# pappuks/medical-image-codec

Hardware: AMD Instinct MI355X
Metric: PICS-8 encode+decode throughput over raw u16 bytes (XR-shaped frames), lossless (higher is better)
Workload: dtype u16; 1 GPU; PICS-8 encode+decode, 288 distinct XR-like 2577x2048 12-bit synthetic frames (2304 strips) per GPU per step, noise tuned to the published XR PICS-8 ratio; frames_per_gpu=288, strips_per_frame=8, width=2577, height=2048, fse=2-state (CompressParallelStrips default), parallelism=1 x independent batches

## Files before the change

### medical-image-codec_amd/csrc/mic_api.hip

```cpp
#include "mic_session.h"

namespace micapi {

std::mutex g_mu;
std::condition_variable g_pool_cv;
int g_device = 0;
std::vector<int> g_devices(1, 0);
bool g_device_ok = false;
std::string g_device_name;
struct DevPool { std::vector<mic_hip_session *> free_; int made = 0; };
std::map<int, DevPool> g_pools;
thread_local mic_hip_session *tl_default = nullptr;
thread_local int tl_depth = 0;

static int pool_max() {
    static const int v = [] { const char *e = getenv("MIC_HIP_POOL"); const int n = e ? atoi(e) : 3; return std::min(std::max(n, 1), 16); }();
    return v;
}

int check_device(int device) {
    static std::mutex mu; static std::vector<int8_t> known;
    std::lock_guard<std::mutex> lk(mu);
    int n = 0;
    if (device < 0 || hipGetDeviceCount(&n) != hipSuccess || device >= n) return MIC_ERR_DEVICE;
// ... 585 lines not shown
    out8[0] = u.ntok; out8[1] = u.blob_len; out8[2] = u.table_log; out8[3] = u.symbol_len;
    out8[4] = u.max_count; out8[5] = u.hdr_len; out8[6] = u.zero_bits; out8[7] = u.flavour;
    out8[8] = u.count; out8[9] = u.bits_off; out8[10] = (uint32_t)u.nstates_used; out8[11] = (uint32_t)u.status; out8[12] = u.nseg; out8[13] = u.nsym; out8[14] = u.seg_cap;
    out8[15] = u.dec_kernel;
    for (int k = 0; k < 16; k++) out8[16 + k] = u.dbg[k];
    return MIC_OK;
} MIC_ABI_CATCH
int mic_hip_debug_split(mic_hip_session *s, int i, uint32_t *out) try {
    if (!s || !out || i < 0 || i >= s->n_last) return MIC_ERR_ARGS;
    for (int k = 0; k < 3; k++) out[k] = s->h_units[(size_t)i].split[k];
    return MIC_OK;
} MIC_ABI_CATCH
int mic_hip_debug_split_config(mic_hip_session *s, uint32_t min_tokens, uint32_t overlap, uint32_t min_bits16) try {
    if (!s || (overlap && (overlap < 64u || (overlap & 63u)))) return MIC_ERR_ARGS;
    if (min_tokens) s->split_cfg.min_tokens = min_tokens;
    if (overlap) s->split_cfg.overlap = overlap;
    if (min_bits16) s->split_cfg.min_bits16 = min_bits16;
    s->dec_classes = mic_hip_session::ClsMemory{};
    return MIC_OK;
} MIC_ABI_CATCH
int mic_hip_debug_split4(mic_hip_session *s, int i, uint32_t *out) try {
    if (!s || !out || i < 0 || i >= s->n_last) return MIC_ERR_ARGS;
    const uint32_t *r = s->h_units[(size_t)i].split;
    const uint32_t m = r[7] == 4u ? ~0u : 0u;
    out[0] = r[0]; out[1] = r[1] & m; out[2] = r[3] & m; out[3] = r[4] & m; out[4] = r[2]; out[5] = r[5] & m; out[6] = r[6] & m;
    return MIC_OK;
} MIC_ABI_CATCH
int mic_hip_debug_split4_config(mic_hip_session *s, uint32_t min_tokens4) try {
    if (!s) return MIC_ERR_ARGS;
    if (min_tokens4) s->split_cfg.min_tokens4 = min_tokens4;
    s->dec_classes = mic_hip_session::ClsMemory{};
    return MIC_OK;
} MIC_ABI_CATCH
int mic_hip_debug_dec_cls(uint32_t flavour, uint32_t table_log, uint32_t zero_bits) { return mic_dec_cls(flavour, table_log, zero_bits); }
int mic_hip_debug_fetch_hist(mic_hip_session *s, int i, void *dst, size_t bytes) try {
    if (!s || i < 0 || i >= s->n_last || bytes > kSym * 4) return MIC_ERR_ARGS;
    HIP_TRY(hipMemcpy(dst, s->h_units[(size_t)i].hist, bytes, hipMemcpyDeviceToHost));
    return MIC_OK;
} MIC_ABI_CATCH
int mic_hip_debug_tok_paths(mic_hip_session *s, int i, uint32_t *out) try {
    if (!s || !out || i < 0 || i >= s->n_last) return MIC_ERR_ARGS;
    for (int k = 0; k < MIC_TK_PATHS; k++) out[k] = s->h_units[(size_t)i].tk_paths[k];
    return MIC_OK;
} MIC_ABI_CATCH
int mic_hip_debug_fetch_tok(mic_hip_session *s, int i, void *dst, size_t n) try {
    if (!s || i < 0 || i >= s->n_last || n > s->h_units[(size_t)i].tok_cap) return MIC_ERR_ARGS;
    HIP_TRY(hipMemcpy(dst, s->h_units[(size_t)i].tok, n * 2, hipMemcpyDeviceToHost));
    return MIC_OK;
} MIC_ABI_CATCH
int mic_hip_debug_tab_route(mic_hip_session *s, int i, uint32_t *out) try {
    if (!s || !out || i < 0 || i >= s->n_last) return MIC_ERR_ARGS;
    *out = s->h_units[(size_t)i].tb_route;
    return MIC_OK;
} MIC_ABI_CATCH
int mic_hip_debug_enc_kernel(mic_hip_session *s, int i, uint32_t *out) try {
    if (!s || !out || i < 0 || i >= s->n_last) return MIC_ERR_ARGS;
    const MicUnit &u = s->h_units[(size_t)i];
    out[0] = u.enc_kernel & 0xFFu; out[1] = u.enc_rounds; out[2] = (u.enc_kernel & MIC_ENC_HANDED) ? 1u : 0u;
    return MIC_OK;
} MIC_ABI_CATCH
int mic_hip_debug_fetch_table(mic_hip_session *s, int i, int which, void *dst, size_t bytes) try {
    if (!s || !dst || i < 0 || i >= s->n_last || which < 0 || which > 4) return MIC_ERR_ARGS;
    const MicUnit &u = s->h_units[(size_t)i];
    const void *slabs[5] = { u.state_tab, u.tt_nb, u.tt_find, u.tab_sym, u.norm };
    if (bytes > (size_t)u.tab_cap * (which == 3 ? 2 : 4)) return MIC_ERR_ARGS;
    { const int arc = s->activate(); if (arc) return arc; }
// ... 81 lines not shown
```

### medical-image-codec_amd/csrc/mic_decode_ls.hip

```cpp
#include <type_traits>
#include "mic_dev.h"
#include "mic_launch.h"
#include "mic_wave.h"
#include "mic_rlewalk.h"

#define LS_RING 0u
#define LS_CLASSES MIC_CLS_CLASSES
template <int TL> struct LsGeom {
    static constexpr int SPW = TL <= 12 ? 4 : TL == 13 ? 3 : TL == 14 ? 2 : 1;
    static constexpr int WAVES = TL <= 12 ? 4 : TL == 13 ? 3 : TL == 16 ? 1 : 2;
    static constexpr int RING_BLOCKS = TL == 16 ? 8 : 4;
    static constexpr int DEPTH = TL == 16 ? 3 : 2;
    static constexpr int RING_BITS = TL == 16 ? 9 : 8;
    static constexpr uint32_t MIRROR = 256u * RING_BLOCKS;
    static constexpr uint32_t STAGE = MIRROR + 16u;
    static constexpr uint32_t TAB = STAGE + 256u;
    static constexpr uint32_t STREAM_BYTES = TAB + (2u << TL);
    static constexpr uint32_t LDS = WAVES * SPW * STREAM_BYTES;
    static_assert(LDS <= 160 * 1024, "one group must fit a CU's LDS");
};
#define LS_TL 13

typedef __attribute__((address_space(3))) uint32_t *ls_l32;
typedef __attribute__((address_space(3))) uint16_t *ls_l16;
typedef const __attribute__((address_space(1))) uint16_t *ls_gcu16;
typedef const __attribute__((address_space(1))) uint32_t *ls_gcu32;
typedef __attribute__((address_space(1))) uint16_t *ls_gu16;
typedef __attribute__((address_space(1))) uint32_t *ls_gu32;
typedef uint32_t ls_v2 __attribute__((ext_vector_type(2)));

template <int CTRL> __device__ __forceinline__ uint32_t ls_dpp(uint32_t v) {
    return (uint32_t)__builtin_amdgcn_update_dpp(0, (int)v, CTRL, 0xF, 0xF, true);
}
#define LS_QP(a, b, c, d) ((a) | ((b) << 2) | ((c) << 4) | ((d) << 6))
#define LS_ROW_SHR(n) (0x110 + (n))
#define LS_ROW_HALF_MIRROR 0x141

__device__ __forceinline__ uint32_t ls_rl(uint32_t v, int lane) { return (uint32_t)__builtin_amdgcn_readlane((int)v, lane); }
__device__ __forceinline__ uint64_t ls_rl64(uint64_t v, int lane) {
    return ((uint64_t)ls_rl((uint32_t)(v >> 32), lane) << 32) | ls_rl((uint32_t)v, lane);
}

#define LS_SPLIT_LIST MIC_CLS_CLASSES
#define LS_RETRY_LIST (MIC_CLS_CLASSES + 1)
#define LS_SPLIT4_LIST (MIC_CLS_CLASSES + 2)
#define LS_LISTS MIC_CLS_LISTS
__global__ void __launch_bounds__(1024) k_dec_classify(MicUnit *units, int n, int *list, int *count, int split, MicSplitCfg cfg) {
    __shared__ uint32_t s_w[16][LS_LISTS];
    __shared__ uint32_t s_base[LS_LISTS];
    const uint32_t tid = threadIdx.x, lane = tid & 63, wave = tid >> 6;
    if (tid < LS_LISTS) s_base[tid] = 0;
    __syncthreads();
    for (int i0 = 0; i0 < n; i0 += 1024) {
        const int i = i0 + (int)tid;
        int cls = -1;
        if (i < n) {
            MicUnit &u = units[i];
            const uint32_t flav = u.flavour, tl = u.table_log;
            const uint32_t ns = (flav == 108) ? 8u : flav;
            if (u.status == MICD_OK && u.ntok == 0 && (ns == 2 || ns == 4 || ns == 8) && tl >= MIC_MIN_TABLELOG && tl <= MIC_MAX_TABLELOG &&
                !(tl == 16 && u.zero_bits)) {
                if (u.bits_off >= u.comp_len) u.status = MICD_ERR_CORRUPT;
                else if (u.comp_len - u.bits_off < (1u << 27)) {
                    if (u.comp_in[u.comp_len - 1] == 0) u.status = MICD_ERR_CORRUPT;
                    else {
                        cls = mic_dec_cls(flav, tl, u.zero_bits);
                        if (cls == 0 && split && mic_split_gate(u, cfg)) cls = u.count >= cfg.min_tokens4 ? LS_SPLIT4_LIST : LS_SPLIT_LIST;
                    }
                }
            }
        }
        uint32_t rank = 0;
#pragma unroll
        for (int c = 0; c < LS_LISTS; c++) {
            const uint64_t m = __ballot(cls == c);
            if (cls == c) rank = (uint32_t)__popcll(m & ((1ull << lane) - 1ull));
            if (lane == 0) s_w[wave][c] = (uint32_t)__popcll(m);
        }
        __syncthreads();
        if (cls >= 0) {
            uint32_t off = s_base[cls];
            for (uint32_t w = 0; w < wave; w++) off += s_w[w][cls];
            list[(size_t)cls * (size_t)n + off + rank] = i;
        }
        __syncthreads();
        if (tid < LS_LISTS) { uint32_t t = 0; for (int w = 0; w < 16; w++) t += s_w[w][tid]; s_base[tid] += t; }
        __syncthreads();
    }
    if (tid < LS_LISTS) count[tid] = (int)s_base[tid];
    if (tid == LS_RETRY_LIST) count[tid] = 0;
}

template <int N, bool ZB, int TL>
__global__ void __launch_bounds__(64 * LsGeom<TL>::WAVES) k_dec_tans_ls(MicUnit *units, const int *list, const int *count_p) {
    constexpr int LS_SPW = LsGeom<TL>::SPW, LS_WAVES = LsGeom<TL>::WAVES;
    constexpr uint32_t LS_STREAM_BYTES = LsGeom<TL>::STREAM_BYTES, LS_STAGE = LsGeom<TL>::STAGE, LS_TAB = LsGeom<TL>::TAB, LS_MIRROR = LsGeom<TL>::MIRROR;
    constexpr int LS_RB = LsGeom<TL>::RING_BLOCKS, LS_DEPTH = LsGeom<TL>::DEPTH, LS_RBITS = LsGeom<TL>::RING_BITS;
    extern __shared__ uint32_t s_mem[];
    const uint32_t lane = threadIdx.x & 63, wv = threadIdx.x >> 6;
    if ((uint32_t)(uintptr_t)(__attribute__((address_space(3))) uint32_t *)s_mem != 0u) return;
// ... 305 lines not shown
            const uint32_t hi = window(q - (int32_t)pre);
            const uint32_t nx = (uint32_t)((((uint64_t)e << 32) | hi) >> (32u - nb));
            st = valid ? nx : st;
            q += (int32_t)ntot;
        }
        __builtin_amdgcn_s_waitcnt(0xC07F);
#pragma unroll
        for (int j = 0; j < LS_SPW; j++) {
            if (!s_have[j]) continue;
            const uint32_t rj = ls_rl(rem, j * LS_LS), done = s_chunks[j] * 128u;
            const uint32_t s2 = *(ls_l32)(uintptr_t)((wv * LS_SPW + (uint32_t)j) * LS_STREAM_BYTES + LS_STAGE + lane * 4);
            const ls_gu16 o = (ls_gu16)(uintptr_t)s_out[j];
            if (2 * lane < rj) o[done + 2 * lane] = (uint16_t)s2;
            if (2 * lane + 1 < rj) o[done + 2 * lane + 1] = (uint16_t)(s2 >> 16);
        }
    }
    if (have && lane % LS_LS == 0 && lane < LS_SPW * LS_LS) {
        MicUnit &uo = units[list[slot0 + (int)g]];
        uo.dec_kernel = 1u + (uint32_t)((TL <= 12 ? 4 : TL - 13) * 6 + (N == 2 ? 0 : N == 4 ? 2 : 4) + (ZB ? 1 : 0));
        if (count == uo.count && q + 32 - (int32_t)(8u * sb) < 0) uo.status = MICD_ERR_CORRUPT;
        else { uo.ntok = count; uo.dec_stage = MIC_STAGE_STATES; }
    }
}

#ifdef LS_STAMP
#define LS_ST_DECL uint64_t stamp[5] = { 0, 0, 0, 0, 0 }, t_prev = __builtin_amdgcn_s_memtime()
#define LS_ST_OUT(parts_) do { if (lane == 0) { MicUnit &ud = units[unit_i]; for (int i_ = 0; i_ < 5; i_++) ud.dbg[i_] = (uint32_t)(stamp[i_] >> 4); \
                                                ud.dbg[5] = ch_end; ud.dbg[6] = (parts_); } } while (0)
#else
#define LS_ST_DECL do { } while (0)
#define LS_ST_OUT(parts_) do { } while (0)
#endif
template <int PARTS> struct LsParts {
    static_assert(PARTS == 2 || PARTS == 4, "eight parts do not fit the sym slab (DESIGN.md section 4)");
    static constexpr int TL = 13, SPW = 3, WAVES = 3;
    static constexpr int CHUNK = 128 / PARTS;
    static constexpr int BLK = 64 / PARTS, BLK_SHIFT = PARTS == 2 ? 5 : 4;
    static constexpr int RING_BLOCKS = 4, DEPTH = 2, RING_BITS = BLK_SHIFT + 2;
    static constexpr uint32_t MIRROR = 4u * BLK * RING_BLOCKS;
    static constexpr uint32_t STAGE = MIRROR + 16u;
    static constexpr uint32_t PART_BYTES = STAGE + 2u * CHUNK;
    static constexpr uint32_t TAB = (uint32_t)PARTS * PART_BYTES;
    static constexpr uint32_t STREAM_BYTES = TAB + (2u << TL);
    static constexpr uint32_t LDS = WAVES * SPW * STREAM_BYTES;
    static_assert(LDS <= 160 * 1024, "one group must fit a CU's LDS");
    static __device__ __forceinline__ uint32_t region(uint32_t sym_cap, uint32_t tok_cap, uint32_t T) {
        const uint32_t slab = min(sym_cap, tok_cap);
        return (PARTS == 2 ? min(slab, T) : slab / (uint32_t)(PARTS - 1)) & ~(uint32_t)(CHUNK - 1);
    }
};

template <int PARTS>
__global__ void __launch_bounds__(64 * LsParts<PARTS>::WAVES) k_dec_tans_ls_parts(MicUnit *units, const int *list, const int *count_p, int *retry_list,
                                                                                int *retry_count, uint32_t overlap) {
    using G = LsParts<PARTS>;
    constexpr int LS_SPW = G::SPW, LS_RBITS = G::RING_BITS, LS_DEPTH = G::DEPTH;
    constexpr bool ZB = false;
    constexpr uint32_t tl = G::TL, size = 1u << tl, SB = G::STREAM_BYTES, PB = G::PART_BYTES, CH = G::CHUNK, BLK = G::BLK, LP = 2u * PARTS;
    extern __shared__ uint32_t s_mem[];
    const uint32_t lane = threadIdx.x & 63, wv = threadIdx.x >> 6;
    if ((uint32_t)(uintptr_t)(__attribute__((address_space(3))) uint32_t *)s_mem != 0u) return;
    const int n_cls = *count_p;
    const int slot0 = __builtin_amdgcn_readfirstlane(((int)blockIdx.x * G::WAVES + (int)wv) * LS_SPW);
    if (slot0 >= n_cls) return;
    const uint32_t k = lane & 1u;
    const bool real = lane < LP * LS_SPW;
    const uint32_t g = real ? lane / LP : 0u, part = real ? (lane >> 1) & (uint32_t)(PARTS - 1) : 0u;
    const bool last_part = part == (uint32_t)(PARTS - 1);
    const bool have = slot0 + (int)g < n_cls;
    const uint32_t gs = have ? g : 0u;
    const int unit_i = list[slot0 + (int)gs];
    const MicUnit &u = units[unit_i];
    const uint32_t T = have ? u.count : 0u;
    const uint32_t bits_off = u.bits_off, len = u.comp_len - bits_off;
    const uint32_t vbase = (wv * LS_SPW + g) * SB + part * PB;
    const uint32_t tbase = (wv * LS_SPW + gs) * SB + G::TAB;
#pragma unroll 1
    for (int j = 0; j < LS_SPW; j++) {
// ... 13 lines not shown
    const uintptr_t addr = (uintptr_t)bs;
    const uint32_t sb = (uint32_t)(addr & 3);
    const uint64_t gaddr = (uint64_t)(addr - sb);
    const uint32_t Lb = 8u * (len - 1) + (uint32_t)(31 - __clz(last));
    const int32_t cur0 = (int32_t)(Lb + 8u * sb);
    const int32_t top_dw = have ? (cur0 - 1) >> 5 : -1;
    const uint32_t Wb = T ? (uint32_t)min((uint64_t)overlap * (uint64_t)Lb / (uint64_t)T, (uint64_t)Lb) : 0u;
    const uint32_t x = (uint32_t)(((uint64_t)Lb + (uint64_t)(PARTS - 1) * (uint64_t)Wb) / (uint32_t)PARTS);
    const uint32_t pm = (uint32_t)((uint64_t)((uint32_t)PARTS - part) * (uint64_t)x - (uint64_t)((uint32_t)(PARTS - 1) - part) * (uint64_t)Wb);
    int32_t q = (part ? (int32_t)(pm + 8u * sb) : cur0) - 32;
    const int32_t qz = (int32_t)(8u * sb) - 32;
    const uint32_t R = G::region(u.sym_cap, u.tok_cap, T);
    bool s_have[LS_SPW];
    __amdgpu_buffer_rsrc_t rs_in[LS_SPW], rs_tok[LS_SPW], rs_scr[LS_SPW];
    uint32_t s_R[LS_SPW];
#pragma unroll
    for (int j = 0; j < LS_SPW; j++) {
        const int src = (int)LP * j;
        s_have[j] = slot0 + j < n_cls;
        s_R[j] = (uint32_t)__builtin_amdgcn_readfirstlane((int)(s_have[j] ? ls_rl(R, src) : 0u));
        const uint32_t in_bytes = (uint32_t)__builtin_amdgcn_readfirstlane((int)(s_have[j] ? ((uint32_t)((int32_t)ls_rl((uint32_t)top_dw, src) + 1)) * 4u : 0u));
        const uint32_t tok_bytes = (uint32_t)__builtin_amdgcn_readfirstlane((int)(s_have[j] ? (ls_rl(T, src) / CH) * CH * 2u : 0u));
        const uint32_t scr_bytes = s_R[j] * 2u * (uint32_t)(PARTS - 1);
        rs_in[j] = __builtin_amdgcn_make_buffer_rsrc((void *)(uintptr_t)ls_rl64(gaddr, src), 0, (int)in_bytes, 0x00020000);
        rs_tok[j] = __builtin_amdgcn_make_buffer_rsrc((void *)(uintptr_t)ls_rl64((uint64_t)(uintptr_t)u.tok, src), 0, (int)tok_bytes, 0x00020000);
        rs_scr[j] = __builtin_amdgcn_make_buffer_rsrc((void *)(uintptr_t)ls_rl64((uint64_t)(uintptr_t)u.sym, src), 0, (int)scr_bytes, 0x00020000);
    }
    const uint32_t up = lane >> G::BLK_SHIFT, lb = lane & (BLK - 1u);
    constexpr uint32_t LS_OOB = 0x7FFFFFF0u;
    auto blk_of = [&](int j, int32_t qq) -> int32_t {
        return (__builtin_amdgcn_ds_bpermute((int)((LP * (uint32_t)j + 2u * up) << 2), qq) >> 5) >> G::BLK_SHIFT;
    };
    auto load_blk = [&](int j, int32_t b) -> uint32_t {
        return __builtin_amdgcn_raw_buffer_load_b32(rs_in[j], (b * (int32_t)BLK + (int32_t)lb) * 4, 0, 2);
    };
    auto store_blk = [&](int j, int32_t b, uint32_t v) {
        const uint32_t rb = (wv * LS_SPW + (uint32_t)j) * SB + up * PB;
        const uint32_t slot = (uint32_t)b & (uint32_t)(G::RING_BLOCKS - 1);
        *(ls_l32)(uintptr_t)(rb + (slot * BLK + lb) * 4) = v;
        if (lb < 2) *(ls_l32)(uintptr_t)(rb + G::MIRROR + lb * 4 + (slot == 0u ? 0u : 8u)) = v;
    };
    uint32_t pf[LS_SPW]; int32_t pfb[LS_SPW];
#pragma unroll
    for (int j = 0; j < LS_SPW; j++) {
        const int32_t b = blk_of(j, q - (int32_t)(2 * tl));
#pragma unroll
        for (int dd = -1; dd < LS_DEPTH; dd++) store_blk(j, b - dd, load_blk(j, b - dd));
        pfb[j] = b - LS_DEPTH;
        pf[j] = load_blk(j, pfb[j]);
    }
    __builtin_amdgcn_s_waitcnt(0xC07F);
    const uint32_t ringb = vbase;
    const uint32_t stgb = vbase + G::STAGE + 2u * k;
    const uint32_t cb = tbase - 2u * size;
    const uint32_t C = 31u - tl;
    auto window = [&](int32_t qq) -> uint32_t {
        const uint32_t a = (__builtin_amdgcn_ubfe((uint32_t)qq, 5, LS_RBITS) << 2) + ringb;
        const uint32_t w0 = *(ls_l32)(uintptr_t)a, w1 = *(ls_l32)(uintptr_t)(a + 4);
        return __builtin_amdgcn_alignbit(w1, w0, (uint32_t)qq);
    };
    auto entry = [&](uint32_t s) -> uint32_t { return *(ls_l16)(uintptr_t)(s * 2 + cb); };
    uint32_t st = size + (window(q - (int32_t)(k * tl)) >> (32u - tl));
    q -= (int32_t)(2 * tl);
    const uint32_t mk1 = k ? ~0u : 0u;
    const uint32_t Wc = (uint32_t)__builtin_amdgcn_readfirstlane((int)(overlap / CH));
    uint32_t maxT = 0;
#pragma unroll
    for (int j = 0; j < LS_SPW; j++) if (s_have[j]) maxT = max(maxT, ls_rl(T, (int)LP * j));
    const uint32_t ch_cap = (uint32_t)__builtin_amdgcn_readfirstlane((int)(maxT / CH + 2u));
    auto own_chunk = [&](uint32_t c) -> bool { return (int32_t)((c - 1u) * CH) <= (int32_t)T; };
    const uint32_t nl = ((lane & ~1u) + 2u) & 63u;
    uint32_t scr0[LS_SPW];
#pragma unroll
    for (int j = 0; j < LS_SPW; j++) scr0[j] = up ? (PARTS > 2 ? (up - 1u) * s_R[j] * 2u : 0u) + lb * 4u : LS_OOB;
    const uint32_t tok0 = up ? LS_OOB : lb * 4u;
    bool handed = false;
    uint32_t m_ab = 0;
    int32_t qlim = last_part ? qz : INT32_MIN;
    int32_t sn_q = q; uint32_t sn_st = st, sn_ch = 0;
    uint32_t ch = 0;
    LS_ST_DECL;
    for (;; ch++) {
        if (ch == Wc) {
            const int32_t qn = __builtin_amdgcn_ds_bpermute((int)(nl << 2), q);
            m_ab = (uint32_t)__builtin_amdgcn_ds_bpermute((int)(nl << 2), (int)st) |
                   ((uint32_t)__builtin_amdgcn_ds_bpermute((int)((nl | 1u) << 2), (int)st) << 16);
            qlim = last_part ? qz : qn;
            handed = true;
        }
        const bool on = own_chunk(ch) & (q > qlim);
        sn_q = on ? q : sn_q; sn_st = on ? st : sn_st; sn_ch = on ? ch : sn_ch;
        asm volatile("" : "+v"(sn_q), "+v"(sn_st), "+v"(sn_ch));
        if (ch >= ch_cap || !__any(on & real & have)) break;
        LS_T(4);
        if constexpr (PARTS == 2) LS_CHUNK2_N("16", "128"); else LS_CHUNK2_N("8", "64");
        LS_T(0);
#pragma unroll
        for (int j = 0; j < LS_SPW; j++) store_blk(j, pfb[j], pf[j]);
        LS_T(1);
#pragma unroll
        for (int j = 0; j < LS_SPW; j++) pfb[j] = blk_of(j, q) - LS_DEPTH;
#pragma unroll
        for (int j = 0; j < LS_SPW; j++) pf[j] = load_blk(j, pfb[j]);
        LS_T(2);
        {
            uint32_t s2[LS_SPW];
#pragma unroll
            for (int j = 0; j < LS_SPW; j++) s2[j] = *(ls_l32)(uintptr_t)((wv * LS_SPW + (uint32_t)j) * SB + up * PB + G::STAGE + lb * 4);
            const uint32_t off = ch * 2u * CH;
#pragma unroll
            for (int j = 0; j < LS_SPW; j++) {
                const bool fits = (ch + 1u) * CH <= s_R[j];
                __builtin_amdgcn_raw_buffer_store_b32(s2[j], rs_tok[j], (int)(tok0 + off), 0, 2);
                __builtin_amdgcn_raw_buffer_store_b32(s2[j], rs_scr[j], (int)(fits ? scr0[j] + off : LS_OOB), 0, 2);
            }
        }
        LS_T(3);
    }
    const uint32_t ch_end = ch;
    LS_ST_OUT((uint32_t)PARTS);
    const uint32_t sn_s1 = (uint32_t)__builtin_amdgcn_ds_bpermute((int)((lane | 1u) << 2), (int)sn_st);
    const uint32_t *grid = (const uint32_t *)(uintptr_t)gaddr;
    auto peek = [&](int32_t qq) -> uint32_t {
        const int32_t d = qq >> 5;
        const uint32_t w0 = (d >= 0 && d <= top_dw) ? grid[d] : 0u, w1 = (d + 1 >= 0 && d + 1 <= top_dw) ? grid[d + 1] : 0u;
        return __builtin_amdgcn_alignbit(w1, w0, (uint32_t)qq);
    };
    auto step = [&](uint32_t &s, int32_t &pos) {
        const uint32_t e = entry(s), nb = (uint32_t)__builtin_clz(e) - C;
        s = (e << nb) | (peek(pos) >> (32u - nb));
        pos -= (int32_t)nb;
    };
    const uint32_t W = Wc * CH;
    uint32_t met = 0, e_p = 0;
    if (real && have && handed && own_chunk(Wc) && k == 0u && !last_part) {
        const int32_t qn = qlim;
        uint32_t s0 = sn_st, s1 = sn_s1, i = sn_ch * CH; int32_t pos = sn_q;
        const uint32_t i_min = part ? W : 0u;
        for (int n = 0; n <= (int)CH && pos >= qn; n++) {
            if (pos == qn) {
                const uint32_t nxt = (i & 1u) ? s1 : s0, oth = (i & 1u) ? s0 : s1;
                if (i >= i_min && (nxt | (oth << 16)) == m_ab) { met = 1u; e_p = i; }
                break;
            }
            if (i & 1u) step(s1, pos); else step(s0, pos);
            i++;
        }
    }
    const uint32_t l0 = lane & ~(LP - 1u), ll = l0 + LP - 2u;
    uint32_t mets[PARTS - 1] = { met }, es[PARTS - 1] = { e_p };
#pragma unroll
    for (int b = 1; b < PARTS - 1; b++) {
        mets[b] = (uint32_t)__builtin_amdgcn_ds_bpermute((int)((l0 + 2u * (uint32_t)b) << 2), (int)met);
        es[b] = (uint32_t)__builtin_amdgcn_ds_bpermute((int)((l0 + 2u * (uint32_t)b) << 2), (int)e_p);
    }
    const uint32_t pl_s0 = (uint32_t)__builtin_amdgcn_ds_bpermute((int)(ll << 2), (int)sn_st);
    const uint32_t pl_s1 = (uint32_t)__builtin_amdgcn_ds_bpermute((int)((ll + 1u) << 2), (int)sn_st);
    const int32_t pl_q = __builtin_amdgcn_ds_bpermute((int)(ll << 2), sn_q);
    const uint32_t pl_ch = (uint32_t)__builtin_amdgcn_ds_bpermute((int)(ll << 2), (int)sn_ch);
    if (!(real && have && lane == l0)) return;
    uint32_t outcome = MIC_SPLIT_DONE, fail = 0, I[3] = { 0u, PARTS > 2 ? 0u : ~0u, PARTS > 2 ? 0u : ~0u };
    {
        uint32_t at = 0;
#pragma unroll
        for (int b = 0; b < PARTS - 1; b++) {
            if (outcome != MIC_SPLIT_DONE) break;
            if (!mets[b]) { outcome = MIC_SPLIT_NOT_MET; fail = (uint32_t)b + 1u; break; }
            at = b ? at + es[b] - W : es[0];
            I[b] = at;
            if (b ? es[b] > R : at > (T / CH) * CH) { outcome = MIC_SPLIT_NO_ROOM; fail = (uint32_t)b + 1u; }
        }
    }
    if (outcome == MIC_SPLIT_DONE) {
        fail = (uint32_t)PARTS;
        if (I[PARTS - 2] > T) outcome = MIC_SPLIT_BAD_COUNT;
        else {
            const uint32_t j_end = T - I[PARTS - 2] + W, js = pl_ch * CH;
            if (j_end > R) outcome = MIC_SPLIT_NO_ROOM;
            else if (j_end > ch_end * CH) outcome = MIC_SPLIT_BAD_COUNT;
            else if (j_end > js) {
                if (j_end - js > CH) outcome = MIC_SPLIT_BAD_COUNT;
                else {
                    uint32_t s0 = pl_s0, s1 = pl_s1; int32_t pos = pl_q;
                    for (uint32_t j = js; j < j_end; j++) { if (j & 1u) step(s1, pos); else step(s0, pos); }
                    if (pos < qz) outcome = MIC_SPLIT_BAD_COUNT;
                }
            }
        }
        if (outcome == MIC_SPLIT_DONE) fail = 0u;
    }
    MicUnit &uo = units[unit_i];
    uo.split[0] = outcome; uo.split[1] = I[0]; uo.split[2] = W; uo.split[3] = I[1]; uo.split[4] = I[2];
    uo.split[5] = R; uo.split[6] = fail; uo.split[7] = (uint32_t)PARTS;
    if (outcome == MIC_SPLIT_DONE) {
        uo.dec_kernel = 1u;
        uo.ntok = T; uo.dec_stage = MIC_STAGE_STATES;
    } else retry_list[atomicAdd(retry_count, 1)] = unit_i;
}

#define TR_THREADS 256
#define TR_TILE ((TR_THREADS - 64) * 8)
#define TR_SEG (TR_TILE / 64)
#define TR_DENSE 6
static_assert(TR_SEG == 24 && TR_SEG * 64 == TR_TILE, "lane = position / 24 below is (position * 2731) >> 16");
template <int TRTL>
__global__ void __launch_bounds__(TR_THREADS) k_dec_translate(MicUnit *units) {
    MicUnit &u = units[blockIdx.x];
    if (u.status != MICD_OK || u.dec_stage != MIC_STAGE_STATES) return;
    if ((TRTL == 13) != (u.table_log <= 13)) return;
    __shared__ uint16_t s_sym[1 << TRTL];
    __shared__ __attribute__((aligned(16))) uint16_t s_tile[2][TR_TILE + 64];
    const uint32_t tid = threadIdx.x, lane = tid & 63, wave = tid >> 6;
    const uint32_t size = 1u << u.table_log, ntok = u.ntok;
    {
        const uint32_t *src = (const uint32_t *)u.tab_sym;
        for (uint32_t i = tid; i < size / 2; i += TR_THREADS) ((uint32_t *)s_sym)[i] = src[i];
    }
    uint16_t *tok = u.tok;
    const bool sp = TRTL == 13 && u.split[0] == MIC_SPLIT_DONE;
    const uint32_t sp_R = u.split[5], sp_W = u.split[2];
    const uint32_t b1 = sp ? u.split[1] : ~0u, b2 = sp ? u.split[3] : ~0u, b3 = sp ? u.split[4] : ~0u;
    const uint32_t o1 = sp_W - b1, o2 = sp_R + sp_W - b2, o3 = 2u * sp_R + sp_W - b3;
    auto seg_of = [&](uint32_t i) -> uint32_t { return (uint32_t)(i >= b1) + (uint32_t)(i >= b2) + (uint32_t)(i >= b3); };
    auto scr_of = [&](uint32_t p, uint32_t i) -> uint32_t { return i + (p == 1u ? o1 : p == 2u ? o2 : o3); };
    const uint16_t *scr = u.sym;
    const bool frame = u.mode == 0 && u.seg != nullptr;
    const bool prefixed = u.mode == 1 && u.walk_mode == 1 && u.seg != nullptr;
    MicRleWalk wk; wk.init(u, frame, ntok);
    bool w_dense = false;
    __syncthreads();
    typedef uint32_t tr_v4 __attribute__((ext_vector_type(4)));
    const uint32_t smask = size - 1;
    for (uint32_t base = 0, it = 0; base < ntok; base += TR_TILE, it++) {
        const uint32_t tile_end = min(base + TR_TILE, ntok);
        uint16_t *tile = s_tile[it & 1];
        if (wave != 0) {
            const uint32_t l = (tid - 64) * 8, i0 = base + l;
            const uint32_t pseg = seg_of(i0);
            if (i0 + 8 <= tile_end && pseg == seg_of(i0 + 7u)) {
                tr_v4 v;
                if (pseg == 0u) v = __builtin_nontemporal_load((const tr_v4 *)(tok + i0));
                else {
                    const uint32_t sj = scr_of(pseg, i0);
                    const uint32_t *d = (const uint32_t *)(scr + (sj & ~1u));
                    const uint32_t sh = (sj & 1u) * 16u;
                    const uint32_t d0 = __builtin_nontemporal_load(d), d1 = __builtin_nontemporal_load(d + 1), d2 = __builtin_nontemporal_load(d + 2),
                                   d3 = __builtin_nontemporal_load(d + 3), d4 = __builtin_nontemporal_load(d + 4);
                    v.x = __builtin_amdgcn_alignbit(d1, d0, sh); v.y = __builtin_amdgcn_alignbit(d2, d1, sh);
                    v.z = __builtin_amdgcn_alignbit(d3, d2, sh); v.w = __builtin_amdgcn_alignbit(d4, d3, sh);
                }
                tr_v4 o;
                o.x = (uint32_t)s_sym[v.x & smask] | ((uint32_t)s_sym[(v.x >> 16) & smask] << 16);
                o.y = (uint32_t)s_sym[v.y & smask] | ((uint32_t)s_sym[(v.y >> 16) & smask] << 16);
                o.z = (uint32_t)s_sym[v.z & smask] | ((uint32_t)s_sym[(v.z >> 16) & smask] << 16);
                o.w = (uint32_t)s_sym[v.w & smask] | ((uint32_t)s_sym[(v.w >> 16) & smask] << 16);
                *(tr_v4 *)(tok + i0) = o;
                *(tr_v4 *)(tile + l) = o;
// ... 92 lines not shown
    uint16_t *tok = u.tok;
    typedef uint32_t tr_v4 __attribute__((ext_vector_type(4)));
    const uint32_t nvec = ntok / 8;
    for (uint32_t i = tid; i < nvec; i += TRW_THREADS) {
        const tr_v4 v = __builtin_nontemporal_load((const tr_v4 *)(tok + 8 * i));
        tr_v4 o;
        o.x = (uint32_t)s_sym[v.x & smask] | ((uint32_t)s_sym[(v.x >> 16) & smask] << 16);
        o.y = (uint32_t)s_sym[v.y & smask] | ((uint32_t)s_sym[(v.y >> 16) & smask] << 16);
        o.z = (uint32_t)s_sym[v.z & smask] | ((uint32_t)s_sym[(v.z >> 16) & smask] << 16);
        o.w = (uint32_t)s_sym[v.w & smask] | ((uint32_t)s_sym[(v.w >> 16) & smask] << 16);
        *(tr_v4 *)(tok + 8 * i) = o;
    }
    for (uint32_t i = 8 * nvec + tid; i < ntok; i += TRW_THREADS) tok[i] = s_sym[tok[i] & smask];
    __syncthreads();
    if (tid == 0) u.dec_stage = MIC_STAGE_PARTS;
}

template <int N, bool ZB, int TL> static void launch_ls_list(MicUnit *d_units, int n, const int *list, const int *count, hipStream_t stream);
template <int N, bool ZB, int TL>
static void launch_ls_class(MicUnit *d_units, int n, const int *d_list, const int *d_count, hipStream_t stream, uint32_t cls_mask) {
    constexpr int cls = (TL <= 12 ? 4 : TL - 13) * 6 + (N == 2 ? 0 : N == 4 ? 2 : 4) + (ZB ? 1 : 0);
    if (!((cls_mask >> cls) & 1u)) return;
    launch_ls_list<N, ZB, TL>(d_units, n, d_list + (size_t)cls * (size_t)n, d_count + cls, stream);
}
template <int N, bool ZB, int TL>
static void launch_ls_list(MicUnit *d_units, int n, const int *list, const int *count, hipStream_t stream) {
    constexpr int per = LsGeom<TL>::WAVES * LsGeom<TL>::SPW;
    static MicPerDeviceOnce once;
    once.run([] { (void)hipFuncSetAttribute((const void *)k_dec_tans_ls<N, ZB, TL>, hipFuncAttributeMaxDynamicSharedMemorySize, LsGeom<TL>::LDS); });
    const unsigned groups = (unsigned)((n + per - 1) / per);
    hipLaunchKernelGGL((k_dec_tans_ls<N, ZB, TL>), dim3(groups), dim3(64 * LsGeom<TL>::WAVES), LsGeom<TL>::LDS, stream, d_units, list, count);
}
template <int PARTS>
static void launch_ls_parts(MicUnit *d_units, int n, int *d_list, int *d_count, int from, hipStream_t stream, uint32_t overlap) {
    using G = LsParts<PARTS>;
    constexpr int per = G::WAVES * G::SPW;
    static MicPerDeviceOnce once;
    once.run([] { (void)hipFuncSetAttribute((const void *)k_dec_tans_ls_parts<PARTS>, hipFuncAttributeMaxDynamicSharedMemorySize, G::LDS); });
    const unsigned groups = (unsigned)((n + per - 1) / per);
    hipLaunchKernelGGL((k_dec_tans_ls_parts<PARTS>), dim3(groups), dim3(64 * G::WAVES), G::LDS, stream, d_units, d_list + (size_t)from * (size_t)n,
                       d_count + from, d_list + (size_t)LS_RETRY_LIST * (size_t)n, d_count + LS_RETRY_LIST, overlap);
}
template <int TL>
static void launch_ls_tl(MicUnit *d_units, int n, const int *d_list, const int *d_count, hipStream_t stream, bool skip_first, uint32_t m) {
    if (!skip_first) launch_ls_class<2, false, TL>(d_units, n, d_list, d_count, stream, m);
    if constexpr (TL < 16) launch_ls_class<2, true, TL>(d_units, n, d_list, d_count, stream, m);
    launch_ls_class<4, false, TL>(d_units, n, d_list, d_count, stream, m);
    if constexpr (TL < 16) launch_ls_class<4, true, TL>(d_units, n, d_list, d_count, stream, m);
    launch_ls_class<8, false, TL>(d_units, n, d_list, d_count, stream, m);
    if constexpr (TL < 16) launch_ls_class<8, true, TL>(d_units, n, d_list, d_count, stream, m);
}

void mic_launch_dec_tans_ls(MicUnit *d_units, int n, int *d_list, int *d_count, hipStream_t stream, MicTimer *t, uint32_t cls_mask, const MicSplitCfg *cfg) {
    const MicSplitCfg sc = cfg ? *cfg : MicSplitCfg{};
    const bool split = (cls_mask & MIC_CLS_SPLIT) != 0;
    if (t) t->mark("k_dec_classify");
    hipLaunchKernelGGL(k_dec_classify, dim3(1), dim3(1024), 0, stream, d_units, n, d_list, d_count, split ? 1 : 0, sc);
    if (split) {
        if (t) t->mark("k_dec_tans_ls_split4<13>");
        launch_ls_parts<4>(d_units, n, d_list, d_count, LS_SPLIT4_LIST, stream, sc.overlap & ~63u);
        if (t) t->mark("k_dec_tans_ls_split<13>");
        launch_ls_parts<2>(d_units, n, d_list, d_count, LS_SPLIT_LIST, stream, sc.overlap & ~63u);
        if (cls_mask & MIC_CLS_RETRY) {
            if (t) t->mark("k_dec_tans_ls<2,false,13> retry");
            launch_ls_list<2, false, 13>(d_units, n, d_list + (size_t)LS_RETRY_LIST * (size_t)n, d_count + LS_RETRY_LIST, stream);
        }
    }
    if (t) t->mark("k_dec_tans_ls<2,false,13>");
    launch_ls_class<2, false, 13>(d_units, n, d_list, d_count, stream, cls_mask);
    if (t) t->mark("k_dec_tans_ls<other,13>");
    launch_ls_tl<13>(d_units, n, d_list, d_count, stream, true, cls_mask);
    if (t) t->mark("k_dec_tans_ls<..12>");
    launch_ls_tl<12>(d_units, n, d_list, d_count, stream, false, cls_mask);
    if (t) t->mark("k_dec_tans_ls<14..16>");
    launch_ls_tl<14>(d_units, n, d_list, d_count, stream, false, cls_mask);
    launch_ls_tl<15>(d_units, n, d_list, d_count, stream, false, cls_mask);
    launch_ls_tl<16>(d_units, n, d_list, d_count, stream, false, cls_mask);
    if (t) t->mark("k_dec_translate");
    if (cls_mask & (0x3F00003Fu | MIC_CLS_SPLIT)) hipLaunchKernelGGL(k_dec_translate<13>, dim3((unsigned)n), dim3(TR_THREADS), 0, stream, d_units);
    if (cls_mask & 0x00FFFFC0u) {
        hipLaunchKernelGGL(k_dec_translate_wide, dim3((unsigned)n), dim3(TRW_THREADS), 0, stream, d_units);
        hipLaunchKernelGGL(k_dec_translate<16>, dim3((unsigned)n), dim3(TR_THREADS), 0, stream, d_units);
    }
}

extern "C" int mic_hip_debug_ls_geom(int table_log, int *spw, int *waves) {
    switch (table_log) {
    case 12: *spw = LsGeom<12>::SPW; *waves = LsGeom<12>::WAVES; return 1;
    case 13: *spw = LsGeom<13>::SPW; *waves = LsGeom<13>::WAVES; return 1;
    case 14: *spw = LsGeom<14>::SPW; *waves = LsGeom<14>::WAVES; return 1;
    case 15: *spw = LsGeom<15>::SPW; *waves = LsGeom<15>::WAVES; return 1;
    case 16: *spw = LsGeom<16>::SPW; *waves = LsGeom<16>::WAVES; return 1;
    }
    return 0;
}
// ... 1 lines not shown
```

### medical-image-codec_amd/csrc/mic_dev.h

```cpp
#pragma once
#include <hip/hip_runtime.h>
#include <stdint.h>

#define MIC_MAXSYM        65535u
#define MIC_MIN_TABLELOG  5
#define MIC_MAX_TABLELOG  16
#define MIC_DEF_TABLELOG  11
#define MIC_GAP_HDR_MAX   8195u
__host__ __device__ inline uint32_t mic_gap_map_off(uint32_t tab_cap) { return 2u * tab_cap; }
__host__ __device__ inline uint32_t mic_gap_stride(uint32_t tab_cap) { return (2u * tab_cap + MIC_GAP_HDR_MAX + 255u) & ~255u; }

#define MICD_OK                  0
#define MICD_ERR_ARGS           -1
#define MICD_ERR_USE_RLE        -3
#define MICD_ERR_CAPACITY       -5
#define MICD_ERR_CORRUPT        -6
#define MICD_ERR_INTERNAL       -8
#define MICD_ERR_UNSUPPORTED    -9
#define MICD_ERR_INCOMPRESSIBLE -10
#define MICD_INT_GROW           -21
#define MICD_GAP_CHECK          -22
#define MIC_DEC_BY_GL           31u
#define MIC_DEC_BY_SERIAL       32u
#define MIC_SPLIT_NOT_TRIED     0u
#define MIC_SPLIT_DONE          1u
#define MIC_SPLIT_NOT_MET       2u
#define MIC_SPLIT_BAD_COUNT     3u
#define MIC_SPLIT_NO_ROOM       4u
struct MicSplitCfg {
    uint32_t min_tokens = 131072u;
    uint32_t overlap = 32768u;
    uint32_t min_bits16 = 144u;
    uint32_t min_tokens4 = 262144u;
};
#define MIC_ENC_BY_SERIAL       8u
#define MIC_ENC_HANDED          0x100u
#define MIC_TKP_FAST            0
#define MIC_TKP_REFUSED         1
#define MIC_TKP_ESC             2
#define MIC_TKP_GENERAL         3
#define MIC_TKP_PERLANE         4
#define MIC_TKP_ROUND2          5
#define MIC_TKP_SERIAL          6
#define MIC_TKP_PACKED          7
#define MIC_TKP_KIND2           8
#define MIC_TK_PATHS            9
#define MIC_TBR_SMALL           (1u << 0)
#define MIC_TBR_HBM             (1u << 1)
#define MIC_TBR_RANS            (1u << 2)
#define MIC_TBR_PRIMARY         (1u << 3)
#define MIC_TBR_N2_PAR          (1u << 4)
#define MIC_TBR_N2_UNIFORM      (1u << 5)
#define MIC_TBR_N2_SERIAL       (1u << 6)
#define MIC_TBR_W_PAR           (1u << 7)
#define MIC_TBR_W_SERIAL        (1u << 8)
#define MIC_TBR_P_SMALL         (1u << 9)
#define MIC_TBR_P_DEFER_TL      (1u << 10)
#define MIC_TBR_P_DEFER_LEN     (1u << 11)
#define MIC_TBR_P_DEFER_SYMS    (1u << 12)
#define MIC_TBR_P_BIG_STAGE     (1u << 13)
#define MIC_TBR_P_BIG_HBM       (1u << 14)
#define MIC_TBR_P_WINDOW        (1u << 15)

enum MicStage : uint32_t {
    MIC_STAGE_NONE   = 0,
    MIC_STAGE_SEGS   = 1,
// ... 36 lines not shown
    uint32_t  nsym;
    uint32_t  dec_stage;
    uint32_t  dec_thr;
    uint32_t  walk_mode;
    uint32_t  wv_slow;
    uint32_t  wv_zmax;
    uint32_t  hist_hi;
    uint32_t  gap;
    uint32_t  gap_hdr_len;
    uint32_t  gap_nsym;
    uint8_t  *gap_buf;
    uint32_t ntok;
    uint32_t blob_len;
    int32_t  status;
    int32_t  nstates_used;
    uint32_t symbol_len;
    uint32_t max_count;
    uint32_t table_log;
    uint32_t zero_bits;
    uint32_t hdr_len;
    uint32_t bits_off;
    uint32_t count;
    uint32_t flavour;
    uint32_t packed_direct;
    uint32_t skip_pack;
    uint32_t dec_kernel;
    uint32_t dbg[16];
    uint32_t tb_route;
    uint32_t tk_paths[MIC_TK_PATHS];
    uint32_t enc_kernel;
    uint32_t enc_rounds;
    uint32_t sym_limit;
    uint32_t split[8];
};
__host__ __device__ inline bool mic_is_prefix(const MicUnit &u) { return u.sym_limit != 0 && u.ntok < u.count; }
__host__ __device__ inline uint32_t mic_sym_ceiling(const MicUnit &u, uint32_t count) {
    if (u.sym_limit == 0 || u.sym_limit > 0xFFFFFF00u) return count;
    const uint32_t c = (u.sym_limit + 127u) & ~127u;
    return c < count ? c : count;
}

struct MicPicaImage {
    uint64_t px_off;
    int32_t  w, h;
    int32_t  nstrips;
    uint32_t rows;
    uint32_t row0;
    uint32_t start0;
};

#define MIC_GLOBAL __attribute__((address_space(1)))
template <class T> using mic_gp = MIC_GLOBAL T *;
template <class T> __device__ __forceinline__ mic_gp<T> mic_g(T *p) { return (mic_gp<T>)p; }

#ifdef MIC_STAMP
#define MIC_STAMP_BEGIN() uint64_t _mic_t0 = __builtin_amdgcn_s_memtime()
#define MIC_STAMP_AT(u, k) do { const uint64_t _t = __builtin_amdgcn_s_memtime(); if (threadIdx.x == 0) (u).dbg[k] += (uint32_t)(_t - _mic_t0); _mic_t0 = _t; } while (0)
#else
#define MIC_STAMP_BEGIN() do { } while (0)
#define MIC_STAMP_AT(u, k) do { } while (0)

#endif

#define MIC_GROUP_HANDOFF() do { asm volatile("s_waitcnt vmcnt(0)" ::: "memory"); __syncthreads(); \
                                 __builtin_amdgcn_fence(__ATOMIC_ACQUIRE, "agent"); } while (0)

// ... 16 lines not shown
```

### medical-image-codec_amd/csrc/mic_launch.h

```cpp
#pragma once
#include <hip/hip_runtime.h>
#include <atomic>
#include <mutex>
#include <vector>
#include "mic_dev.h"

struct MicPerDeviceOnce {
    std::atomic<uint64_t> mask{0};
    std::mutex mu;
    template <class F> void run(F &&setup) {
        int d = 0;
        if (hipGetDevice(&d) != hipSuccess) { setup(); return; }
        const uint64_t bit = 1ull << (d & 63);
        if (mask.load(std::memory_order_acquire) & bit) return;
        std::lock_guard<std::mutex> lk(mu);
        if (mask.load(std::memory_order_relaxed) & bit) return;
        setup();
        mask.fetch_or(bit, std::memory_order_release);
    }
};

struct MicTimer {
    bool enabled = false;
    bool accumulate = false;
    hipStream_t stream = nullptr;
    std::vector<hipEvent_t> pool;
    std::vector<const char *> names;
    size_t used = 0;
    void reset(hipStream_t s) { stream = s; if (!accumulate) { used = 0; names.clear(); } }
    void clear() { used = 0; names.clear(); }
    void mark(const char *name) {
        if (!enabled) return;
        if (used == pool.size()) { hipEvent_t e; if (hipEventCreate(&e) != hipSuccess) return; pool.push_back(e); }
        (void)hipEventRecord(pool[used++], stream);
        names.push_back(name);
    }
    void destroy() { for (auto e : pool) (void)hipEventDestroy(e); pool.clear(); used = 0; names.clear(); }
};

#define MIC_VARIANT_GRAD 0x1000
#define MIC_VARIANT_NARROW 0x2000
#define MIC_VARIANT_FRAMES 0x4000
#define MIC_VARIANT_GAP 0x8000
#define MIC_ENC_CLS_NARROW2 0x01u
#define MIC_ENC_CLS_WIDE    0x02u
#define MIC_ENC_CLS_SMALL12 0x04u
#define MIC_ENC_CLS_SMALL13 0x08u
#define MIC_ENC_CLS_TL14    0x10u
#define MIC_ENC_CLS_TL15    0x20u
#define MIC_ENC_CLS_TL16    0x40u
void mic_launch_encode(MicUnit *d_units, int n, hipStream_t stream, int variant, MicTimer *t, uint32_t enc_mask = ~0u);
#define MIC_CLS_HEAD 64
#define MIC_CLS_CLASSES 30
#define MIC_CLS_LISTS 33
#define MIC_CLS_INTS(n) (MIC_CLS_HEAD + MIC_CLS_LISTS * (size_t)(n))
#define MIC_CLS_SPLIT 0x40000000u
#define MIC_CLS_RETRY 0x80000000u
void mic_launch_decode(MicUnit *d_units, int n, hipStream_t stream, int variant, MicTimer *t, int *d_cls, uint32_t pred_mask = ~0u, uint32_t cls_mask = ~0u,
                       const MicSplitCfg *split = nullptr);
void mic_launch_dec_tans_ls(MicUnit *d_units, int n, int *d_list, int *d_count, hipStream_t stream, MicTimer *t, uint32_t cls_mask = ~0u,
                            const MicSplitCfg *split = nullptr);
void mic_launch_pack(const MicUnit *d_units, int n, uint64_t *d_off, uint8_t *d_dst, uint64_t d_cap, hipStream_t stream, MicTimer *t);
void mic_launch_pica_bounds(const uint16_t *d_px, const MicPicaImage *d_tab, int nimg, uint32_t rows, unsigned long long *d_cost,
                            int32_t *d_starts, hipStream_t stream, MicTimer *t);
void mic_launch_pica_pick(MicUnit *d_units, int npairs, hipStream_t stream, MicTimer *t);
#define MIC_PRED_NARROW 0x100u
#define MIC_PRED_WAVE2  0x200u
#define MIC_PRED_WIDE   0x400u
void mic_launch_decode_pixels(MicUnit *d_units, int n, hipStream_t stream, MicTimer *t, bool any_grad = false, uint32_t pred_mask = ~0u);
void mic_launch_decode_rows(MicUnit *d_units, int n, hipStream_t stream, uint32_t kmask);
void mic_launch_decode_fused(MicUnit *d_units, int n, hipStream_t stream, uint32_t kmask);
#define MIC_ROWS_LO 1008
#define MIC_ROWS_HI 2688
__host__ __device__ inline int mic_rows_k(int w) {
    if (w <= MIC_ROWS_LO || w > MIC_ROWS_HI) return 0;
    const int k = (w + 63) >> 6;
    return 18 + 4 * ((max(k, 18) - 18 + 3) / 4);
}
__host__ __device__ inline uint32_t mic_rows_kbit(int w) { const int k = mic_rows_k(w); return k ? 1u << ((k - 18) / 4) : 0u; }
__host__ __device__ inline uint32_t mic_pred_bit(int w) {
    return w <= MIC_ROWS_LO ? MIC_PRED_NARROW : w <= MIC_ROWS_HI ? mic_rows_kbit(w) : w <= 8192 - 64 ? MIC_PRED_WAVE2 : MIC_PRED_WIDE;
}
__host__ __device__ inline int mic_dec_cls(uint32_t flavour, uint32_t tl, uint32_t zero_bits) {
    const uint32_t ns = flavour == 108 ? 8u : flavour;
    if (!(ns == 2 || ns == 4 || ns == 8) || tl < MIC_MIN_TABLELOG || tl > MIC_MAX_TABLELOG || (tl == 16 && zero_bits)) return -1;
    return (tl <= 12 ? 4 : (int)tl - 13) * 6 + (ns == 2 ? 0 : ns == 4 ? 2 : 4) + (zero_bits ? 1 : 0);
}
// ... 12 lines not shown
```

Measured before the change: 174.4 GB/s.

## Add eight-part split decode for large 2-state tl13 units

Adds an 8-part split variant of the tANS split decoder for the largest qualifying units (count ≥ min_tokens8), which cascades failures to the 4-part list and then to the retry list. Eight parts use smaller ring blocks, skip writing the warm-up region to scratch, and use different buffer cache flags. The transpose/scatter stage gets extra boundaries for the additional segments. This aims to expose more parallelism per long serial stream, at the cost of more overlap work, extra boundary checks, and another kernel launch.

Result: faster. 186.4 GB/s, median of 6 (+6.9%).

```diff
diff --git a/medical-image-codec_amd/csrc/mic_api.hip b/medical-image-codec_amd/csrc/mic_api.hip
--- a/medical-image-codec_amd/csrc/mic_api.hip
+++ b/medical-image-codec_amd/csrc/mic_api.hip
@@ -641,6 +641,22 @@
     s->dec_classes = mic_hip_session::ClsMemory{};
     return MIC_OK;
 } MIC_ABI_CATCH
+int mic_hip_debug_split8(mic_hip_session *s, int i, uint32_t *out) try {
+    if (!s || !out || i < 0 || i >= s->n_last) return MIC_ERR_ARGS;
+    const MicUnit &u = s->h_units[(size_t)i];
+    const uint32_t *r = u.split;
+    const uint32_t m = r[7] == 8u ? ~0u : 0u;
+    out[0] = r[0]; out[1] = r[1] & m; out[2] = r[3] & m; out[3] = r[4] & m;
+    for (int k = 0; k < 4; k++) out[4 + k] = u.split_hi[k] & m;
+    out[8] = r[2]; out[9] = r[5] & m; out[10] = r[6] & m; out[11] = r[7];
+    return MIC_OK;
+} MIC_ABI_CATCH
+int mic_hip_debug_split8_config(mic_hip_session *s, uint32_t min_tokens8) try {
+    if (!s) return MIC_ERR_ARGS;
+    if (min_tokens8) s->split_cfg.min_tokens8 = min_tokens8;
+    s->dec_classes = mic_hip_session::ClsMemory{};
+    return MIC_OK;
+} MIC_ABI_CATCH
 int mic_hip_debug_dec_cls(uint32_t flavour, uint32_t table_log, uint32_t zero_bits) { return mic_dec_cls(flavour, table_log, zero_bits); }
 int mic_hip_debug_fetch_hist(mic_hip_session *s, int i, void *dst, size_t bytes) try {
     if (!s || i < 0 || i >= s->n_last || bytes > kSym * 4) return MIC_ERR_ARGS;
diff --git a/medical-image-codec_amd/csrc/mic_decode_ls.hip b/medical-image-codec_amd/csrc/mic_decode_ls.hip
--- a/medical-image-codec_amd/csrc/mic_decode_ls.hip
+++ b/medical-image-codec_amd/csrc/mic_decode_ls.hip
@@ -44,6 +44,7 @@
 #define LS_SPLIT_LIST MIC_CLS_CLASSES
 #define LS_RETRY_LIST (MIC_CLS_CLASSES + 1)
 #define LS_SPLIT4_LIST (MIC_CLS_CLASSES + 2)
+#define LS_SPLIT8_LIST (MIC_CLS_CLASSES + 3)
 #define LS_LISTS MIC_CLS_LISTS
 __global__ void __launch_bounds__(1024) k_dec_classify(MicUnit *units, int n, int *list, int *count, int split, MicSplitCfg cfg) {
     __shared__ uint32_t s_w[16][LS_LISTS];
@@ -65,7 +66,8 @@
                     if (u.comp_in[u.comp_len - 1] == 0) u.status = MICD_ERR_CORRUPT;
                     else {
                         cls = mic_dec_cls(flav, tl, u.zero_bits);
-                        if (cls == 0 && split && mic_split_gate(u, cfg)) cls = u.count >= cfg.min_tokens4 ? LS_SPLIT4_LIST : LS_SPLIT_LIST;
+                        if (cls == 0 && split && mic_split_gate(u, cfg))
+                            cls = u.count >= max(cfg.min_tokens8, cfg.min_tokens4) ? LS_SPLIT8_LIST : u.count >= cfg.min_tokens4 ? LS_SPLIT4_LIST : LS_SPLIT_LIST;
                     }
                 }
             }
@@ -437,10 +439,10 @@
 #define LS_ST_OUT(parts_) do { } while (0)
 #endif
 template <int PARTS> struct LsParts {
-    static_assert(PARTS == 2 || PARTS == 4, "eight parts do not fit the sym slab (DESIGN.md section 4)");
+    static_assert(PARTS == 2 || PARTS == 4 || PARTS == 8, "a part needs a ring block of at least 8 dwords: a chunk of 128 / PARTS symbols must not cross two");
     static constexpr int TL = 13, SPW = 3, WAVES = 3;
     static constexpr int CHUNK = 128 / PARTS;
-    static constexpr int BLK = 64 / PARTS, BLK_SHIFT = PARTS == 2 ? 5 : 4;
+    static constexpr int BLK = 64 / PARTS, BLK_SHIFT = PARTS == 2 ? 5 : PARTS == 4 ? 4 : 3;
     static constexpr int RING_BLOCKS = 4, DEPTH = 2, RING_BITS = BLK_SHIFT + 2;
     static constexpr uint32_t MIRROR = 4u * BLK * RING_BLOCKS;
     static constexpr uint32_t STAGE = MIRROR + 16u;
@@ -449,6 +451,8 @@
     static constexpr uint32_t STREAM_BYTES = TAB + (2u << TL);
     static constexpr uint32_t LDS = WAVES * SPW * STREAM_BYTES;
     static_assert(LDS <= 160 * 1024, "one group must fit a CU's LDS");
+    static constexpr bool SKIP_W = PARTS == 8;
+    static constexpr int AUX = PARTS == 8 ? 0 : 2;
     static __device__ __forceinline__ uint32_t region(uint32_t sym_cap, uint32_t tok_cap, uint32_t T) {
         const uint32_t slab = min(sym_cap, tok_cap);
         return (PARTS == 2 ? min(slab, T) : slab / (uint32_t)(PARTS - 1)) & ~(uint32_t)(CHUNK - 1);
@@ -528,7 +532,7 @@
         return (__builtin_amdgcn_ds_bpermute((int)((LP * (uint32_t)j + 2u * up) << 2), qq) >> 5) >> G::BLK_SHIFT;
     };
     auto load_blk = [&](int j, int32_t b) -> uint32_t {
-        return __builtin_amdgcn_raw_buffer_load_b32(rs_in[j], (b * (int32_t)BLK + (int32_t)lb) * 4, 0, 2);
+        return __builtin_amdgcn_raw_buffer_load_b32(rs_in[j], (b * (int32_t)BLK + (int32_t)lb) * 4, 0, G::AUX);
     };
     auto store_blk = [&](int j, int32_t b, uint32_t v) {
         const uint32_t rb = (wv * LS_SPW + (uint32_t)j) * SB + up * PB;
@@ -589,7 +593,7 @@
         asm volatile("" : "+v"(sn_q), "+v"(sn_st), "+v"(sn_ch));
         if (ch >= ch_cap || !__any(on & real & have)) break;
         LS_T(4);
-        if constexpr (PARTS == 2) LS_CHUNK2_N("16", "128"); else LS_CHUNK2_N("8", "64");
+        if constexpr (PARTS == 2) LS_CHUNK2_N("16", "128"); else if constexpr (PARTS == 4) LS_CHUNK2_N("8", "64"); else LS_CHUNK2_N("4", "32");
         LS_T(0);
 #pragma unroll
         for (int j = 0; j < LS_SPW; j++) store_blk(j, pfb[j], pf[j]);
@@ -604,11 +608,12 @@
 #pragma unroll
             for (int j = 0; j < LS_SPW; j++) s2[j] = *(ls_l32)(uintptr_t)((wv * LS_SPW + (uint32_t)j) * SB + up * PB + G::STAGE + lb * 4);
             const uint32_t off = ch * 2u * CH;
+            const uint32_t ch0 = G::SKIP_W ? Wc : 0u, soff = (ch - ch0) * 2u * CH;
 #pragma unroll
             for (int j = 0; j < LS_SPW; j++) {
-                const bool fits = (ch + 1u) * CH <= s_R[j];
-                __builtin_amdgcn_raw_buffer_store_b32(s2[j], rs_tok[j], (int)(tok0 + off), 0, 2);
-                __builtin_amdgcn_raw_buffer_store_b32(s2[j], rs_scr[j], (int)(fits ? scr0[j] + off : LS_OOB), 0, 2);
+                const bool fits = ch >= ch0 && (ch + 1u - ch0) * CH <= s_R[j];
+                __builtin_amdgcn_raw_buffer_store_b32(s2[j], rs_tok[j], (int)(tok0 + off), 0, G::AUX);
+                __builtin_amdgcn_raw_buffer_store_b32(s2[j], rs_scr[j], (int)(fits ? scr0[j] + soff : LS_OOB), 0, G::AUX);
             }
         }
         LS_T(3);
@@ -655,7 +660,11 @@
     const int32_t pl_q = __builtin_amdgcn_ds_bpermute((int)(ll << 2), sn_q);
     const uint32_t pl_ch = (uint32_t)__builtin_amdgcn_ds_bpermute((int)(ll << 2), (int)sn_ch);
     if (!(real && have && lane == l0)) return;
-    uint32_t outcome = MIC_SPLIT_DONE, fail = 0, I[3] = { 0u, PARTS > 2 ? 0u : ~0u, PARTS > 2 ? 0u : ~0u };
+    constexpr int NI = PARTS > 4 ? PARTS - 1 : 3;
+    uint32_t outcome = MIC_SPLIT_DONE, fail = 0, I[NI];
+#pragma unroll
+    for (int b = 0; b < NI; b++) I[b] = b && PARTS == 2 ? ~0u : 0u;
+    const uint32_t dead = G::SKIP_W ? W : 0u;
     {
         uint32_t at = 0;
 #pragma unroll
@@ -664,7 +673,7 @@
             if (!mets[b]) { outcome = MIC_SPLIT_NOT_MET; fail = (uint32_t)b + 1u; break; }
             at = b ? at + es[b] - W : es[0];
             I[b] = at;
-            if (b ? es[b] > R : at > (T / CH) * CH) { outcome = MIC_SPLIT_NO_ROOM; fail = (uint32_t)b + 1u; }
+            if (b ? es[b] - dead > R : at > (T / CH) * CH) { outcome = MIC_SPLIT_NO_ROOM; fail = (uint32_t)b + 1u; }
         }
     }
     if (outcome == MIC_SPLIT_DONE) {
@@ -672,7 +681,7 @@
         if (I[PARTS - 2] > T) outcome = MIC_SPLIT_BAD_COUNT;
         else {
             const uint32_t j_end = T - I[PARTS - 2] + W, js = pl_ch * CH;
-            if (j_end > R) outcome = MIC_SPLIT_NO_ROOM;
+            if (j_end - dead > R) outcome = MIC_SPLIT_NO_ROOM;
             else if (j_end > ch_end * CH) outcome = MIC_SPLIT_BAD_COUNT;
             else if (j_end > js) {
                 if (j_end - js > CH) outcome = MIC_SPLIT_BAD_COUNT;
@@ -688,6 +697,7 @@
     MicUnit &uo = units[unit_i];
     uo.split[0] = outcome; uo.split[1] = I[0]; uo.split[2] = W; uo.split[3] = I[1]; uo.split[4] = I[2];
     uo.split[5] = R; uo.split[6] = fail; uo.split[7] = (uint32_t)PARTS;
+    if constexpr (PARTS == 8) { uo.split_hi[0] = I[3]; uo.split_hi[1] = I[4]; uo.split_hi[2] = I[5]; uo.split_hi[3] = I[6]; }
     if (outcome == MIC_SPLIT_DONE) {
         uo.dec_kernel = 1u;
         uo.ntok = T; uo.dec_stage = MIC_STAGE_STATES;
@@ -713,12 +723,19 @@
         for (uint32_t i = tid; i < size / 2; i += TR_THREADS) ((uint32_t *)s_sym)[i] = src[i];
     }
     uint16_t *tok = u.tok;
-    const bool sp = TRTL == 13 && u.split[0] == MIC_SPLIT_DONE;
-    const uint32_t sp_R = u.split[5], sp_W = u.split[2];
+    const bool sp = TRTL == 13 && u.split[0] == MIC_SPLIT_DONE, sp8 = sp && u.split[7] == 8u;
+    const uint32_t sp_R = u.split[5], sp_W = sp8 ? 0u : u.split[2];
     const uint32_t b1 = sp ? u.split[1] : ~0u, b2 = sp ? u.split[3] : ~0u, b3 = sp ? u.split[4] : ~0u;
+    const uint32_t b4 = sp8 ? u.split_hi[0] : ~0u, b5 = sp8 ? u.split_hi[1] : ~0u, b6 = sp8 ? u.split_hi[2] : ~0u, b7 = sp8 ? u.split_hi[3] : ~0u;
     const uint32_t o1 = sp_W - b1, o2 = sp_R + sp_W - b2, o3 = 2u * sp_R + sp_W - b3;
-    auto seg_of = [&](uint32_t i) -> uint32_t { return (uint32_t)(i >= b1) + (uint32_t)(i >= b2) + (uint32_t)(i >= b3); };
-    auto scr_of = [&](uint32_t p, uint32_t i) -> uint32_t { return i + (p == 1u ? o1 : p == 2u ? o2 : o3); };
+    const uint32_t o4 = 3u * sp_R - b4, o5 = 4u * sp_R - b5, o6 = 5u * sp_R - b6, o7 = 6u * sp_R - b7;
+    auto seg_of = [&](uint32_t i) -> uint32_t {
+        return (uint32_t)(i >= b1) + (uint32_t)(i >= b2) + (uint32_t)(i >= b3) + (uint32_t)(i >= b4) + (uint32_t)(i >= b5) + (uint32_t)(i >= b6) +
+               (uint32_t)(i >= b7);
+    };
+    auto scr_of = [&](uint32_t p, uint32_t i) -> uint32_t {
+        return i + (p == 1u ? o1 : p == 2u ? o2 : p == 3u ? o3 : p == 4u ? o4 : p == 5u ? o5 : p == 6u ? o6 : o7);
+    };
     const uint16_t *scr = u.sym;
     const bool frame = u.mode == 0 && u.seg != nullptr;
     const bool prefixed = u.mode == 1 && u.walk_mode == 1 && u.seg != nullptr;
@@ -877,14 +894,14 @@
     hipLaunchKernelGGL((k_dec_tans_ls<N, ZB, TL>), dim3(groups), dim3(64 * LsGeom<TL>::WAVES), LsGeom<TL>::LDS, stream, d_units, list, count);
 }
 template <int PARTS>
-static void launch_ls_parts(MicUnit *d_units, int n, int *d_list, int *d_count, int from, hipStream_t stream, uint32_t overlap) {
+static void launch_ls_parts(MicUnit *d_units, int n, int *d_list, int *d_count, int from, int to, hipStream_t stream, uint32_t overlap) {
     using G = LsParts<PARTS>;
     constexpr int per = G::WAVES * G::SPW;
     static MicPerDeviceOnce once;
     once.run([] { (void)hipFuncSetAttribute((const void *)k_dec_tans_ls_parts<PARTS>, hipFuncAttributeMaxDynamicSharedMemorySize, G::LDS); });
     const unsigned groups = (unsigned)((n + per - 1) / per);
     hipLaunchKernelGGL((k_dec_tans_ls_parts<PARTS>), dim3(groups), dim3(64 * G::WAVES), G::LDS, stream, d_units, d_list + (size_t)from * (size_t)n,
-                       d_count + from, d_list + (size_t)LS_RETRY_LIST * (size_t)n, d_count + LS_RETRY_LIST, overlap);
+                       d_count + from, d_list + (size_t)to * (size_t)n, d_count + to, overlap);
 }
 template <int TL>
 static void launch_ls_tl(MicUnit *d_units, int n, const int *d_list, const int *d_count, hipStream_t stream, bool skip_first, uint32_t m) {
@@ -902,10 +919,12 @@
     if (t) t->mark("k_dec_classify");
     hipLaunchKernelGGL(k_dec_classify, dim3(1), dim3(1024), 0, stream, d_units, n, d_list, d_count, split ? 1 : 0, sc);
     if (split) {
+        if (t) t->mark("k_dec_tans_ls_split8<13>");
+        launch_ls_parts<8>(d_units, n, d_list, d_count, LS_SPLIT8_LIST, LS_SPLIT4_LIST, stream, sc.overlap & ~63u);
         if (t) t->mark("k_dec_tans_ls_split4<13>");
-        launch_ls_parts<4>(d_units, n, d_list, d_count, LS_SPLIT4_LIST, stream, sc.overlap & ~63u);
+        launch_ls_parts<4>(d_units, n, d_list, d_count, LS_SPLIT4_LIST, LS_RETRY_LIST, stream, sc.overlap & ~63u);
         if (t) t->mark("k_dec_tans_ls_split<13>");
-        launch_ls_parts<2>(d_units, n, d_list, d_count, LS_SPLIT_LIST, stream, sc.overlap & ~63u);
+        launch_ls_parts<2>(d_units, n, d_list, d_count, LS_SPLIT_LIST, LS_RETRY_LIST, stream, sc.overlap & ~63u);
         if (cls_mask & MIC_CLS_RETRY) {
             if (t) t->mark("k_dec_tans_ls<2,false,13> retry");
             launch_ls_list<2, false, 13>(d_units, n, d_list + (size_t)LS_RETRY_LIST * (size_t)n, d_count + LS_RETRY_LIST, stream);
diff --git a/medical-image-codec_amd/csrc/mic_dev.h b/medical-image-codec_amd/csrc/mic_dev.h
--- a/medical-image-codec_amd/csrc/mic_dev.h
+++ b/medical-image-codec_amd/csrc/mic_dev.h
@@ -32,6 +32,7 @@
     uint32_t overlap = 32768u;
     uint32_t min_bits16 = 144u;
     uint32_t min_tokens4 = 262144u;
+    uint32_t min_tokens8 = 393216u;
 };
 #define MIC_ENC_BY_SERIAL       8u
 #define MIC_ENC_HANDED          0x100u
@@ -134,6 +135,7 @@
     uint32_t enc_rounds;
     uint32_t sym_limit;
     uint32_t split[8];
+    uint32_t split_hi[4];
 };
 __host__ __device__ inline bool mic_is_prefix(const MicUnit &u) { return u.sym_limit != 0 && u.ntok < u.count; }
 __host__ __device__ inline uint32_t mic_sym_ceiling(const MicUnit &u, uint32_t count) {
diff --git a/medical-image-codec_amd/csrc/mic_launch.h b/medical-image-codec_amd/csrc/mic_launch.h
--- a/medical-image-codec_amd/csrc/mic_launch.h
+++ b/medical-image-codec_amd/csrc/mic_launch.h
@@ -52,7 +52,7 @@
 void mic_launch_encode(MicUnit *d_units, int n, hipStream_t stream, int variant, MicTimer *t, uint32_t enc_mask = ~0u);
 #define MIC_CLS_HEAD 64
 #define MIC_CLS_CLASSES 30
-#define MIC_CLS_LISTS 33
+#define MIC_CLS_LISTS 34
 #define MIC_CLS_INTS(n) (MIC_CLS_HEAD + MIC_CLS_LISTS * (size_t)(n))
 #define MIC_CLS_SPLIT 0x40000000u
 #define MIC_CLS_RETRY 0x80000000u
```
